# Adamtaranto/frisk

Hardware: NVIDIA B200
Metric: Gbp/s scaffold scored (k-mer count+window score) (higher is better)
Workload: dtype u4/u16/u64 counts + f64 scores

## Files before the change

### frisk_b200/csrc/frisk_tables.cu

```cuda
#include <cooperative_groups.h>
#include <cuda_runtime.h>
#include <math_constants.h>
#include <stdint.h>

#include <atomic>

#include "../../include/frisk_b200.h"
#include "frisk_internal.h"
#include "frisk_device.cuh"

namespace {

constexpr int kThreads = 1024;

__device__ __forceinline__ uint32_t revcomp_idx(uint32_t idx, int x) {
    uint32_t r = __brev(idx) >> (32 - 2 * x);
    r = ((r >> 1) & 0x55555555u) | ((r & 0x55555555u) << 1);
    return r ^ (0x55555555u & (pow4(x) - 1u));
}

__device__ __noinline__ void bg_wrapped(unsigned long long* __restrict__ fwd_k, uint32_t code, uint32_t old) {
    atomicAdd(&fwd_k[code], 65536ull);
    if (!(code & 1u))
        atomicAdd(&fwd_k[code | 1u], old == 0xffffffffu ? 65535ull : ~0ull);
}

__device__ __forceinline__ void bg_add(uint32_t* tab, unsigned long long* __restrict__ fwd_k, uint32_t code) {
    const uint32_t sh = (code & 1u) * 16u;
    const uint32_t old = atomicAdd(&tab[code >> 1], 1u << sh);
    if (((old >> sh) & 0xffffu) == 0xffffu) bg_wrapped(fwd_k, code, old);
}

__device__ __forceinline__ uint32_t bg_room(uint32_t old, uint32_t sh) { return ~(old | (0xffff0000u >> sh)); }

template <int K>
__global__ void __launch_bounds__(kThreads, 1)
bg_count_kernel(const uint32_t* __restrict__ codes, const uint32_t* __restrict__ inv, const uint32_t* __restrict__ low,
                uint64_t word_lo, uint64_t word_hi, int mask_host, unsigned long long* __restrict__ fwd,
                uint32_t* __restrict__ partial, const unsigned long long* __restrict__ d_range) {
    constexpr uint32_t NB = pow4(K);
    constexpr uint32_t NW = NB / 2u;
    extern __shared__ __align__(16) uint32_t tab[];
    if (d_range) { word_lo = d_range[0]; word_hi = d_range[1]; }
    const uint64_t n_words = word_hi - word_lo;
    const uint64_t per = (n_words + gridDim.x - 1) / gridDim.x;
    const uint64_t w0 = word_lo + per * blockIdx.x;
    uint64_t w1 = w0 + per;
    if (w1 > word_hi) w1 = word_hi;
    const bool use_low = mask_host && low != nullptr;
    unsigned long long* fwd_k = fwd + lvl_off(K);

    for (uint32_t b = threadIdx.x; b < NW; b += kThreads) tab[b] = 0;
    __syncthreads();
    for (uint64_t wd = w0 + threadIdx.x; wd < w1; wd += kThreads) {
        uint32_t m0 = __ldg(inv + wd), m1 = __ldg(inv + wd + 1);
        if (use_low) { m0 |= __ldg(low + wd); m1 |= __ldg(low + wd + 1); }
        const uint32_t c0 = __ldg(codes + 2 * wd), c1 = __ldg(codes + 2 * wd + 1), c2 = __ldg(codes + 2 * wd + 2);
        const bool all_valid = (m0 == 0u) && (K == 1 || (m1 >> ((33 - K) & 31)) == 0u);
        if (all_valid) {
            uint32_t olds[32], room = 0xffffffffu;
#pragma unroll
            for (int p = 0; p < 32; ++p) {
                const uint32_t code = (p < 16 ? __funnelshift_l(c1, c0, 2 * p) : __funnelshift_l(c2, c1, 2 * (p - 16)))
                                      >> (32 - 2 * K);
                const uint32_t sh = (code & 1u) * 16u;
                olds[p] = atomicAdd(&tab[code >> 1], 1u << sh);
                room = min(room, bg_room(olds[p], sh));
            }
            if (room == 0u) {
#pragma unroll 1
                for (int p = 0; p < 32; ++p) {
                    const uint32_t code = (p < 16 ? __funnelshift_l(c1, c0, 2 * p) : __funnelshift_l(c2, c1, 2 * (p - 16)))
                                          >> (32 - 2 * K);
                    uint32_t old = 0;
#pragma unroll
                    for (int q = 0; q < 32; ++q) if (q == p) old = olds[q];
                    if (bg_room(old, (code & 1u) * 16u) == 0u) bg_wrapped(fwd_k, code, old);
                }
            }
        } else {
#pragma unroll 4
            for (int p = 0; p < 32; ++p) {
                const uint32_t code = (p < 16 ? __funnelshift_l(c1, c0, 2 * p) : __funnelshift_l(c2, c1, 2 * (p - 16)))
                                      >> (32 - 2 * K);
                const int v = min(__clz(__funnelshift_l(m1, m0, p)), K);
                if (v == K) bg_add(tab, fwd_k, code);
                else if (v > 0) atomicAdd(&fwd[lvl_off(v) + (code >> (2 * (K - v)))], 1ull);
            }
        }
    }
    __syncthreads();
    if (partial) {
        uint32_t* dst = partial + (size_t)blockIdx.x * NW;
        if constexpr (NW >= 4u * kThreads) {
            for (uint32_t b = threadIdx.x * 4u; b < NW; b += kThreads * 4u)
                *reinterpret_cast<uint4*>(dst + b) = *reinterpret_cast<const uint4*>(tab + b);
        } else {
            for (uint32_t b = threadIdx.x; b < NW; b += kThreads) dst[b] = tab[b];
        }
    } else {
        for (uint32_t b = threadIdx.x; b < NW; b += kThreads) {
            const uint32_t c = tab[b];
            if (c & 0xffffu) atomicAdd(&fwd_k[2u * b], (unsigned long long)(c & 0xffffu));
            if (c >> 16) atomicAdd(&fwd_k[2u * b + 1u], (unsigned long long)(c >> 16));
        }
    }
}

template <int K>
__global__ void __launch_bounds__(256)
bg_reduce_kernel(const uint32_t* __restrict__ partial, int n_parts, unsigned long long* __restrict__ fwd) {
    constexpr uint32_t NW = pow4(K) / 2u;
    __shared__ unsigned long long acc[8][32][2];
    const uint32_t lane = threadIdx.x & 31u, warp = threadIdx.x >> 5;
    const uint32_t w = blockIdx.x * 32u + lane;
    unsigned long long lo = 0, hi = 0;
    if (w < NW) {
#pragma unroll 4
        for (int c = (int)warp; c < n_parts; c += 8) {
            const uint32_t v = partial[(size_t)c * NW + w];
            lo += v & 0xffffu;
            hi += v >> 16;
        }
    }
    acc[warp][lane][0] = lo; acc[warp][lane][1] = hi;
    __syncthreads();
    if (warp == 0 && w < NW) {
#pragma unroll
        for (int j = 1; j < 8; ++j) { lo += acc[j][lane][0]; hi += acc[j][lane][1]; }
        if (lo) fwd[lvl_off(K) + 2u * w] += lo;
        if (hi) fwd[lvl_off(K) + 2u * w + 1u] += hi;
    }
}

struct LocalFwd {
    const unsigned long long* p;
    const long long* space_dev = nullptr;
    __device__ __forceinline__ unsigned long long operator()(uint32_t i) const { return p[i]; }
    __device__ __forceinline__ void arrive_and_wait() const {}
    __device__ __forceinline__ long long space(long long by_value) const { return space_dev ? *space_dev : by_value; }
};
using frisk_internal::kMaxPeers;
struct PeerFwd {
    const unsigned long long* p[kMaxPeers];
    unsigned long long* flags[kMaxPeers];
    int n, rank;
    unsigned long long epoch;
    __device__ __forceinline__ long long space(long long by_value) const { return by_value; }
    __device__ __forceinline__ unsigned long long operator()(uint32_t i) const {
        unsigned long long v[kMaxPeers];
#pragma unroll
        for (int q = 0; q < kMaxPeers; ++q) v[q] = q < n ? __ldcv(p[q] + i) : 0ull;
        unsigned long long s = 0;
#pragma unroll
        for (int q = 0; q < kMaxPeers; ++q) s += v[q];
        return s;
    }
    __device__ __forceinline__ void arrive_and_wait() const {
        if (epoch == 0) return;
        if (blockIdx.x == 0 && (int)threadIdx.x < n) {
            __threadfence_system();
            asm volatile("st.release.sys.global.u64 [%0], %1;" ::"l"(flags[threadIdx.x] + rank), "l"(epoch) : "memory");
        }
        if (threadIdx.x == 0) {
            const long long t0 = clock64();
            for (int q = 0; q < n; ++q) {
                unsigned long long seen;
                do {
                    asm volatile("ld.acquire.sys.global.u64 %0, [%1];" : "=l"(seen) : "l"(flags[rank] + q) : "memory");
                    if (seen < epoch && clock64() - t0 > 20000000000ll) __trap();
                } while (seen < epoch);
            }
        }
        __syncthreads();
    }
};

template <int K, typename Fwd>
__device__ __forceinline__ void forward_totals_body(const Fwd& fwd, unsigned long long* __restrict__ tables,
                                                    unsigned long long* __restrict__ valid_kmax, uint32_t root,
                                                    unsigned long long (*lvl)[256], unsigned long long* red) {
    constexpr int R = K > 4 ? K - 4 : 0;
    const uint32_t t = threadIdx.x;
    uint32_t n = pow4(K - R);
    constexpr int LV = K - (R > 1 ? R : 1);
    unsigned long long own[LV > 0 ? LV : 1];
    unsigned long long v = 0;
    if (t < n) v = fwd(lvl_off(K) + root * n + t);
    {
        uint32_t m = n;
#pragma unroll
        for (int i = 0; i < LV; ++i) {
            m >>= 2;
            own[i] = (t < m) ? fwd(lvl_off(K - 1 - i) + root * m + t) : 0ull;
        }
    }
    if (t < n) {
        tables[lvl_off(K) + root * n + t] = v;
        lvl[0][t] = v;
    }
    unsigned long long local = v;
    for (int o = 16; o; o >>= 1) local += __shfl_xor_sync(kFull, local, o);
    if ((t & 31) == 0) red[t >> 5] = local;
    __syncthreads();
    if (t == 0 && valid_kmax) {
        unsigned long long sum = 0;
        for (int w = 0; w < 8; ++w) sum += red[w];
        if (sum) atomicAdd(valid_kmax, sum);
    }
    int cur = 0;
#pragma unroll
    for (int i = 0; i < LV; ++i) {
        const int x = K - 1 - i;
        n >>= 2;
        if (t < n) {
            const unsigned long long* ch = &lvl[cur][4 * t];
            const unsigned long long f = own[i] + ch[0] + ch[1] + ch[2] + ch[3];
            tables[lvl_off(x) + root * n + t] = f;
            lvl[cur ^ 1][t] = f;
        }
        cur ^= 1;
        __syncthreads();
    }
}

template <int K, typename Fwd>
__global__ void __launch_bounds__(256)
forward_totals_kernel(const Fwd fwd, unsigned long long* __restrict__ tables,
                      unsigned long long* __restrict__ valid_kmax) {
    __shared__ unsigned long long lvl[2][256];
    __shared__ unsigned long long red[8];
    fwd.arrive_and_wait();
    forward_totals_body<K, Fwd>(fwd, tables, valid_kmax, blockIdx.x, lvl, red);
}

template <int K, typename Fwd>
__device__ __forceinline__ void forward_low_body(const Fwd& fwd, unsigned long long* __restrict__ tables) {
    constexpr int R = K > 4 ? K - 4 : 0;
    const uint32_t t = threadIdx.x;
    unsigned long long own[R > 1 ? R - 1 : 1];
#pragma unroll
    for (int x = R - 1; x >= 1; --x) own[x - 1] = (t < pow4(x)) ? fwd(lvl_off(x) + t) : 0ull;
#pragma unroll
    for (int x = R - 1; x >= 1; --x) {
        if (t < pow4(x)) {
            const unsigned long long* ch = tables + lvl_off(x + 1) + 4 * t;
            tables[lvl_off(x) + t] = own[x - 1] + __ldcg(ch) + __ldcg(ch + 1) + __ldcg(ch + 2) + __ldcg(ch + 3);
        }
        __syncthreads();
    }
}

template <int K, typename Fwd>
__global__ void __launch_bounds__(64)
forward_low_kernel(const Fwd fwd, unsigned long long* __restrict__ tables) {
    forward_low_body<K, Fwd>(fwd, tables);
}

template <int K>
__device__ __forceinline__ void symmetrise_entry(unsigned long long* __restrict__ tables, uint32_t i) {
    int x = 1;
#pragma unroll
    for (int y = 2; y <= K; ++y) x += (i >= lvl_off(y));
    const uint32_t b = i - lvl_off(x);
    const uint32_t r = revcomp_idx(b, x);
    if (b < r) {
        const unsigned long long sum = __ldcg(tables + i) + __ldcg(tables + lvl_off(x) + r);
        tables[i] = sum;
        tables[lvl_off(x) + r] = sum;
    } else if (b == r) {
        tables[i] = 2ull * __ldcg(tables + i);
    }
}

template <int K>
__global__ void __launch_bounds__(256)
symmetrise_kernel(unsigned long long* __restrict__ tables) {
    const uint32_t i = blockIdx.x * 256 + threadIdx.x;
    if (i < lvl_off(K + 1)) symmetrise_entry<K>(tables, i);
}

template <int K>
__device__ __forceinline__ void genome_ivom_entry(const unsigned long long* __restrict__ tables, int kmin, long long space,
                                                  double2* __restrict__ ig, uint32_t kappa) {
    double num = 0.0;
    unsigned long long den = 0;
    bool bad = false;
#pragma unroll
    for (int x = 1; x <= K; ++x) {
        if (x < kmin) continue;
        const unsigned long long c = __ldcg(tables + lvl_off(x) + (kappa >> (2 * (K - x))));
        const long long d = (space - (long long)(x - 1)) * 2;
        if (d == 0) bad = true;
        const double q = (double)pow4(x) / (double)d;
        const double cd = (double)c;
        num = fma(q, cd * cd, num);
        den += c << (2 * x);
        if (x == kmin && c == 0) bad = true;
    }
    double v = bad ? CUDART_NAN : num / (double)den;
    ig[kappa] = make_double2(v, log2(v));
}

template <int K>
__global__ void genome_ivom_kernel(const unsigned long long* __restrict__ tables, int kmin, long long space,
                                   double2* __restrict__ ig) {
    const uint32_t kappa = blockIdx.x * blockDim.x + threadIdx.x;
    if (kappa < pow4(K)) genome_ivom_entry<K>(tables, kmin, space, ig, kappa);
}

template <int K, typename Fwd>
__global__ void __launch_bounds__(256)
finalize_ivom_kernel(const Fwd fwd, unsigned long long* __restrict__ tables, unsigned long long* __restrict__ valid_kmax,
                     int kmin, long long space, double2* __restrict__ ig) {
    namespace cg = cooperative_groups;
    cg::grid_group grid = cg::this_grid();
    constexpr int R = K > 4 ? K - 4 : 0;
    __shared__ unsigned long long lvl[2][256];
    __shared__ unsigned long long red[8];
    fwd.arrive_and_wait();
    for (uint32_t root = blockIdx.x; root < pow4(R); root += gridDim.x) {
        forward_totals_body<K, Fwd>(fwd, tables, valid_kmax, root, lvl, red);
        __syncthreads();
    }
    grid.sync();
    if (R > 1) {
        if (blockIdx.x == 0) forward_low_body<K, Fwd>(fwd, tables);
        grid.sync();
    }
    const uint32_t gtid = blockIdx.x * 256 + threadIdx.x, gstride = gridDim.x * 256;
    for (uint32_t i = gtid; i < lvl_off(K + 1); i += gstride) symmetrise_entry<K>(tables, i);
    grid.sync();
    const long long sp = fwd.space(space);
    for (uint32_t kappa = gtid; kappa < pow4(K); kappa += gstride) genome_ivom_entry<K>(tables, kmin, sp, ig, kappa);
}

using frisk_internal::check_k;
using frisk_internal::sm_count_cached;
#define CK(call) FRISK_CK(call)

template <int K>
int launch_background(const uint32_t* codes, const uint32_t* inv, const uint32_t* low, uint64_t w_lo, uint64_t w_hi,
                      int mask_host, uint64_t* fwd, cudaStream_t st, const unsigned long long* d_range = nullptr) {
    constexpr uint32_t NB = pow4(K);
    constexpr uint32_t NW = NB / 2u;
    const size_t smem = (size_t)NW * 4;
    CK(cudaFuncSetAttribute(bg_count_kernel<K>, cudaFuncAttributeMaxDynamicSharedMemorySize, (int)smem));
    const uint64_t n_words = w_hi - w_lo;
    int grid = sm_count_cached();
    if (grid <= 0) return FRISK_E_NO_DEVICE;
    const uint64_t want = (n_words + 2047) / 2048;
    if ((uint64_t)grid > want) grid = want ? (int)want : 1;
    uint32_t* partial = nullptr;
    if (NB >= 4096u && grid > 1) {
        int rc = frisk_internal::pool_ready();
        if (rc) return rc;
        CK(cudaMallocAsync((void**)&partial, (size_t)grid * NW * sizeof(uint32_t), st));
    }
    bg_count_kernel<K><<<grid, kThreads, smem, st>>>(codes, inv, low, w_lo, w_hi, mask_host,
                                                      reinterpret_cast<unsigned long long*>(fwd), partial, d_range);
    if (partial) {
        bg_reduce_kernel<K><<<(NW + 31) / 32, 256, 0, st>>>(partial, grid, reinterpret_cast<unsigned long long*>(fwd));
        CK(cudaFreeAsync(partial, st));
    }
    CK(cudaGetLastError());
    return FRISK_OK;
}

template <int K, typename Fwd>
int launch_finalize(const Fwd f, int symmetric, uint64_t* tables, uint64_t* valid, cudaStream_t st) {
    constexpr int R = K > 4 ? K - 4 : 0;
    auto t = reinterpret_cast<unsigned long long*>(tables);
    if (valid) CK(cudaMemsetAsync(valid, 0, sizeof(uint64_t), st));
    forward_totals_kernel<K, Fwd><<<pow4(R), 256, 0, st>>>(f, t, reinterpret_cast<unsigned long long*>(valid));
    if (R > 1) forward_low_kernel<K, Fwd><<<1, 64, 0, st>>>(f, t);
    if (symmetric) symmetrise_kernel<K><<<(lvl_off(K + 1) + 255) / 256, 256, 0, st>>>(t);
    CK(cudaGetLastError());
    return FRISK_OK;
}

template <int K, typename Fwd>
int launch_finalize_ivom(Fwd f, int kmin, int64_t space, uint64_t* tables, uint64_t* valid, double* ig, cudaStream_t st) {
    auto kern = finalize_ivom_kernel<K, Fwd>;
    static std::atomic<int> cached[64];
    int dev = 0;
    CK(cudaGetDevice(&dev));
    int per_sm = cached[dev & 63].load(std::memory_order_acquire);
    if (per_sm == 0) {
        CK(cudaOccupancyMaxActiveBlocksPerMultiprocessor(&per_sm, kern, 256, 0));
        if (per_sm > 0) cached[dev & 63].store(per_sm, std::memory_order_release);
    }
    const int sms = sm_count_cached();
    if (sms <= 0) return FRISK_E_NO_DEVICE;
    if (per_sm < 1) return FRISK_E_UNSUPPORTED;
    int grid = sms * (per_sm > 2 ? 2 : per_sm);
    if (valid) CK(cudaMemsetAsync(valid, 0, sizeof(uint64_t), st));
    unsigned long long* t = reinterpret_cast<unsigned long long*>(tables);
    unsigned long long* v = reinterpret_cast<unsigned long long*>(valid);
    long long sp = (long long)space;
    double2* g = reinterpret_cast<double2*>(ig);
    void* args[] = {(void*)&f, (void*)&t, (void*)&v, (void*)&kmin, (void*)&sp, (void*)&g};
    CK(cudaLaunchCooperativeKernel((const void*)kern, dim3((unsigned)grid), dim3(256), args, 0, st));
    return FRISK_OK;
}

template <int K>
int launch_genome_ivom(const uint64_t* tables, int kmin, int64_t space, double* ig, cudaStream_t st) {
    const uint32_t n = pow4(K);
    const int bs = 256;
    genome_ivom_kernel<K><<<(n + bs - 1) / bs, bs, 0, st>>>(reinterpret_cast<const unsigned long long*>(tables), kmin,
                                                           (long long)space, reinterpret_cast<double2*>(ig));
    CK(cudaGetLastError());
    return FRISK_OK;
}

int peer_fwd(const uint64_t* const* d_fwd_peers, uint64_t* const* d_flag_peers, int rank, int world, uint64_t epoch, PeerFwd* f) {
    if (world > kMaxPeers) return FRISK_E_UNSUPPORTED;
    f->n = world;
    f->rank = rank;
    f->epoch = d_flag_peers ? epoch : 0;
    for (int q = 0; q < kMaxPeers; ++q) { f->p[q] = nullptr; f->flags[q] = nullptr; }
    for (int q = 0; q < world; ++q) {
        if (!d_fwd_peers[q] || (d_flag_peers && !d_flag_peers[q])) return FRISK_E_INVALID;
        f->p[q] = reinterpret_cast<const unsigned long long*>(d_fwd_peers[q]);
        if (d_flag_peers) f->flags[q] = reinterpret_cast<unsigned long long*>(d_flag_peers[q]);
    }
    return FRISK_OK;
}

}

int frisk_internal::finalize_ivom(const uint64_t* d_fwd, const uint64_t* const* d_fwd_peers, uint64_t* const* d_flag_peers, int rank,
                                  int world, uint64_t epoch, int kmin, int kmax, int64_t space, const long long* space_dev,
                                  uint64_t* tables, uint64_t* valid, double* ig, cudaStream_t st) {
    int rc;
    if (kmax > FRISK_B200_FAST_K) {
        if (world > 0 || space_dev) return FRISK_E_UNSUPPORTED;
        if ((rc = frisk_internal::general_finalize(d_fwd, kmax, 1, tables, valid, st))) return rc;
        return frisk_internal::general_genome_ivom(tables, kmin, kmax, space, ig, st);
    }
    if (world == 0) {
        const LocalFwd f{reinterpret_cast<const unsigned long long*>(d_fwd), space_dev};
        DISPATCH_K(kmax, (launch_finalize_ivom<K, LocalFwd>(f, kmin, space, tables, valid, ig, st)));
    }
    if (space_dev) return FRISK_E_UNSUPPORTED;
    PeerFwd f;
    if ((rc = peer_fwd(d_fwd_peers, d_flag_peers, rank, world, epoch, &f))) return rc;
    DISPATCH_K(kmax, (launch_finalize_ivom<K, PeerFwd>(f, kmin, space, tables, valid, ig, st)));
}

extern "C" {

int frisk_b200_background(const uint32_t* d_codes, const uint32_t* d_inv, const uint32_t* d_low, uint64_t first_base,
                          uint64_t last_base, int kmax, int mask_host, uint64_t* d_fwd, void* stream) {
    if (!d_codes || !d_inv || !d_fwd || (first_base & 31) || (last_base & 31) || last_base < first_base)
        return FRISK_E_INVALID;
    int rc = check_k(1, kmax);
    if (rc) return rc;
    if (last_base == first_base) return FRISK_OK;
    cudaStream_t st = (cudaStream_t)stream;
    if (kmax > FRISK_B200_FAST_K)
        return frisk_internal::general_background(d_codes, d_inv, d_low, first_base >> 5, last_base >> 5, kmax, mask_host, d_fwd, st);
    DISPATCH_K(kmax, launch_background<K>(d_codes, d_inv, d_low, first_base >> 5, last_base >> 5, mask_host, d_fwd, st));
}

}

int frisk_internal::background_device_range(const uint32_t* codes, const uint32_t* inv, const uint32_t* low,
                                            const unsigned long long* d_word_range, uint64_t words_hint, int kmax, int mask_host,
                                            uint64_t* fwd, cudaStream_t st) {
    if (!codes || !inv || !fwd || !d_word_range) return FRISK_E_INVALID;
    int rc = check_k(1, kmax);
    if (rc) return rc;
    if (kmax > FRISK_B200_FAST_K) return FRISK_E_UNSUPPORTED;
    DISPATCH_K(kmax, launch_background<K>(codes, inv, low, 0, words_hint ? words_hint : 1, mask_host, fwd, st, d_word_range));
}

extern "C" {

int frisk_b200_finalize_tables(const uint64_t* d_fwd, int kmax, int symmetric, uint64_t* d_tables, uint64_t* d_valid_kmax,
                               void* stream) {
    if (!d_fwd || !d_tables) return FRISK_E_INVALID;
    int rc = check_k(1, kmax);
    if (rc) return rc;
    cudaStream_t st = (cudaStream_t)stream;
    if (kmax > FRISK_B200_FAST_K) return frisk_internal::general_finalize(d_fwd, kmax, symmetric, d_tables, d_valid_kmax, st);
    const LocalFwd f{reinterpret_cast<const unsigned long long*>(d_fwd)};
    DISPATCH_K(kmax, (launch_finalize<K, LocalFwd>(f, symmetric, d_tables, d_valid_kmax, st)));
}

int frisk_b200_finalize_tables_peers(const uint64_t* const* d_fwd_peers, uint64_t* const* d_flag_peers, int rank, int world,
                                     uint64_t epoch, int kmax, int symmetric, uint64_t* d_tables, uint64_t* d_valid_kmax,
                                     void* stream) {
    if (!d_fwd_peers || !d_tables || world < 1 || rank < 0 || rank >= world) return FRISK_E_INVALID;
    if (d_flag_peers && epoch == 0) return FRISK_E_INVALID;
    int rc = check_k(1, kmax);
    if (rc) return rc;
    if (kmax > FRISK_B200_FAST_K) return FRISK_E_UNSUPPORTED;
    PeerFwd f;
    if ((rc = peer_fwd(d_fwd_peers, d_flag_peers, rank, world, epoch, &f))) return rc;
    cudaStream_t st = (cudaStream_t)stream;
    DISPATCH_K(kmax, (launch_finalize<K, PeerFwd>(f, symmetric, d_tables, d_valid_kmax, st)));
}

int frisk_b200_finalize_ivom(const uint64_t* d_fwd, const uint64_t* const* d_fwd_peers, uint64_t* const* d_flag_peers, int rank,
                             int world, uint64_t epoch, int kmin, int kmax, int64_t genome_space, uint64_t* d_tables,
                             uint64_t* d_valid_kmax, double* d_ig, void* stream) {
    if (!d_tables || !d_ig || (world == 0 && !d_fwd) || (world > 0 && (!d_fwd_peers || rank < 0 || rank >= world)))
        return FRISK_E_INVALID;
    if (world > 0 && d_flag_peers && epoch == 0) return FRISK_E_INVALID;
    int rc = check_k(kmin, kmax);
    if (rc) return rc;
    return frisk_internal::finalize_ivom(d_fwd, d_fwd_peers, d_flag_peers, rank, world, epoch, kmin, kmax, genome_space, nullptr,
                                         d_tables, d_valid_kmax, d_ig, (cudaStream_t)stream);
}

int frisk_b200_genome_ivom(const uint64_t* d_tables, int kmin, int kmax, int64_t genome_space, double* d_ig, void* stream) {
    if (!d_tables || !d_ig) return FRISK_E_INVALID;
    int rc = check_k(kmin, kmax);
    if (rc) return rc;
    cudaStream_t st = (cudaStream_t)stream;
    if (kmax > FRISK_B200_FAST_K) return frisk_internal::general_genome_ivom(d_tables, kmin, kmax, genome_space, d_ig, st);
    DISPATCH_K(kmax, launch_genome_ivom<K>(d_tables, kmin, genome_space, d_ig, st));
}

}
```

### frisk_b200/engine.py

```python
from __future__ import annotations

import ctypes as C
import sys
from dataclasses import dataclass, field
from typing import List, Optional, Sequence, Tuple, Union

import numpy as np

from . import _lib

SeqLike = Union[np.ndarray, bytes, str]


def _torch_loaded() -> bool:
    return "torch" in sys.modules


class DevBuf:

    def __init__(self, nbytes: int):
        p = C.c_void_p()
        _lib.check(_lib.lib().frisk_b200_device_alloc(C.byref(p), int(nbytes)), "frisk_b200_device_alloc")
        self._p, self.nbytes = p, int(nbytes)

# ... 507 lines not shown
        _lib.check(_lib.lib().frisk_b200_score(_ptr(dg.codes), _ptr(dg.inv), _ptr(dg.low), _ptr(d_off), _ptr(d_len), n,
                                               wins.max_len, _ptr(d_ig), kmin, kmax, int(rip), _ptr(d_rows),
                                               _ptr(d_status), _ptr(d_dump), _stream_ptr(dev)), "frisk_b200_score")
    return d_rows, d_status, d_dump


_SLOT_CACHE = {}


def feature_slots(kmin: int, kmax: int) -> Tuple[np.ndarray, int]:
    key = (kmin, kmax)
    if key not in _SLOT_CACHE:
        slot = np.zeros(_lib.table_size(1, kmax), np.int32)
        n = C.c_uint64(0)
        _lib.check(_lib.lib().frisk_b200_feature_slots(kmin, kmax, _ptr(slot), C.byref(n)), "frisk_b200_feature_slots")
        _SLOT_CACHE[key] = (slot, int(n.value))
    return _SLOT_CACHE[key]


def region_features(dg: DeviceGenome, off: np.ndarray, length: np.ndarray, kmin: int = 1, kmax: int = 6) -> np.ndarray:
    import torch
    _lib.require_device()
    slot, nf = feature_slots(kmin, kmax)
    n = len(off)
    dev = dg.device
    d_out = torch.empty((n, nf), dtype=torch.float64, device=dev)
    if n:
        d_off = torch.from_numpy(np.ascontiguousarray(off, np.uint64).view(np.int64)).to(dev)
        d_len = torch.from_numpy(np.ascontiguousarray(length, np.uint32).view(np.int32)).to(dev)
        d_slot = torch.from_numpy(slot).to(dev)
        with torch.cuda.device(dev):
            _lib.check(_lib.lib().frisk_b200_region_features(_ptr(dg.codes), _ptr(dg.inv), _ptr(d_off), _ptr(d_len), n, kmin, kmax,
                                                             _ptr(d_slot), nf, _ptr(d_out), _stream_ptr(dev)),
                       "frisk_b200_region_features")
    return d_out.cpu().numpy()


@dataclass
class HotPathResult:
    kmin: int
    kmax: int
    tables: np.ndarray
    meta: Tuple[int, int, int]
    names: List[str]
    coords: np.ndarray
    rows: np.ndarray
    status: np.ndarray
    n_candidates: int = 0
    win_index: np.ndarray = field(default_factory=lambda: np.zeros(0, np.int64))
    row_scaf: np.ndarray = field(default_factory=lambda: np.zeros(0, np.int64))
    win_tables: Optional[np.ndarray] = None
    collective: str = ""
    scaf_names: List[str] = field(default_factory=list)

    def tsv_body(self, with_rip: bool) -> bytes:
        n = len(self.rows)
        enc = [s.encode() for s in self.scaf_names]
        lens = np.array([len(b) for b in enc], dtype=np.uint32)
        offs = (np.cumsum(lens, dtype=np.uint64) - lens).astype(np.uint64)
        blob = np.frombuffer(b"".join(enc) or b"\0", dtype=np.uint8)
        row_name = np.ascontiguousarray(self.row_scaf, dtype=np.uint32)
        start = np.ascontiguousarray(self.coords[:, 0], dtype=np.int64)
        stop = np.ascontiguousarray(self.coords[:, 1], dtype=np.int64)
        rows = np.ascontiguousarray(self.rows, dtype=np.float64)
        nv = 5 if with_rip else 2
        cap = int(lens[row_name].sum()) + n * (44 + 26 * nv) + 16 if n else 16
        out = np.empty(cap, dtype=np.uint8)
        nb = C.c_uint64(0)
        _lib.check(_lib.lib().frisk_b200_format_rows(_ptr(blob), _ptr(offs), _ptr(lens), _ptr(row_name), _ptr(start), _ptr(stop),
                                                     _ptr(rows), n, nv, _ptr(out), cap, C.byref(nb), 0), "frisk_b200_format_rows")
        return out[:int(nb.value)].tobytes()

    def raise_reference_errors(self) -> None:
        bad = np.nonzero(self.status & (_lib.ROW_KLD_ZERODIV | _lib.ROW_GC_ZERODIV))[0]
        if bad.size:
            i = int(bad[0])
            raise ZeroDivisionError("window %s:%d-%d: float division by zero (reference F:437/F:136)"
                                    % (self.names[i], self.coords[i, 0], self.coords[i, 1]))
        bad = np.nonzero(self.status & _lib.ROW_LOG_DOMAIN)[0]
        if bad.size:
            raise ValueError("math domain error (reference F:470)")


def _slice_orders(tab: np.ndarray, kmin: int, kmax: int) -> np.ndarray:
    return tab[..., _lib.table_size(1, kmin - 1):_lib.table_size(1, kmax)] if kmin > 1 else tab[..., :_lib.table_size(1, kmax)]


def assemble(query: PackedGenome, host: PackedGenome, wins: WindowList, tables_1k: np.ndarray, valid_kmax: int,
             rows: np.ndarray, status: np.ndarray, kmin: int, kmax: int, dump: Optional[np.ndarray] = None,
             names: bool = True) -> HotPathResult:
    keep = (status & _lib.ROW_EXCLUDED) == 0
    n_all = len(status)
    if bool(keep.all()):
        idx = np.arange(n_all, dtype=np.int64)
        take = lambda a: np.array(a[:n_all], copy=True)
    else:
        idx = np.nonzero(keep)[0]
        take = lambda a: a[idx]
    want_names = bool(names)
    scaf = take(wins.scaf)
    names = [query.names[s] for s in scaf] if want_names else []
    if idx.size:
        coords = np.empty((idx.size, 2), np.int64)
        coords[:, 0] = take(wins.start)
        coords[:, 1] = take(wins.stop)
    else:
        coords = np.zeros((0, 2), np.int64)
    meta = (host.total_len, host.ex_max(kmax, valid_kmax), host.nn_total)
    wt = None
    if dump is not None:
        wt = _slice_orders(take(dump), kmin, kmax)
    return HotPathResult(kmin, kmax, _slice_orders(tables_1k, kmin, kmax).copy(), meta, names, coords,
                         take(rows), take(status).astype(np.uint32, copy=False), len(wins), idx, scaf.astype(np.int64), wt,
                         scaf_names=list(query.names) if want_names else query.names)


class Pipeline:

    def __init__(self, query: PackedGenome, host: Optional[PackedGenome] = None, kmin: int = 1, kmax: int = 8,
                 w: int = 5000, step: int = 2500, mask_host: bool = False, scaffolds_all: bool = False,
                 rip: bool = True, device="cuda:0", dump: bool = False, allreduce=None,
                 genome_space: Optional[int] = None, wins: Optional[WindowList] = None,
                 bg_range: Optional[Tuple[int, int]] = None, peers=None):
        import torch
        _lib.require_device()
        rc = 0 if 1 <= kmin <= kmax else _lib.E_INVALID
        if kmax > _lib.MAX_K:
            rc = _lib.E_UNSUPPORTED
        _lib.check(rc, "frisk_b200 Pipeline(kmin=%d, kmax=%d)" % (kmin, kmax))
        host = host if host is not None else query
        self.dq = query if isinstance(query, DeviceGenome) else DeviceGenome(query, device)
        self.dh = self.dq if host is query else (host if isinstance(host, DeviceGenome) else DeviceGenome(host, device))
        query, host = self.dq.host, self.dh.host
        self.query, self.host = query, host
        self.kmin, self.kmax, self.mask_host, self.rip = kmin, kmax, mask_host, rip
        self.allreduce = allreduce
        self.peers = peers if (peers is not None and peers.available) else None
        self.genome_space = self.host.genome_space if genome_space is None else int(genome_space)
        self.wins = wins if wins is not None else query.windows(w, step, scaffolds_all)
        self.bg_range = (0, host.padded_len - 32) if bg_range is None else (int(bg_range[0]), int(bg_range[1]))
        dev = self.dq.device
        self.device = dev
        n = len(self.wins)
        tsz = _lib.table_size(1, kmax)
        self.d_fwd = torch.zeros(tsz, dtype=torch.int64, device=dev)
        self.d_tables = torch.empty(tsz, dtype=torch.int64, device=dev)
        self.d_valid = torch.zeros(1, dtype=torch.int64, device=dev)
        self.d_ig = torch.empty(2 * 4 ** kmax, dtype=torch.float64, device=dev)
        self.d_rows = torch.empty((n, 5), dtype=torch.float64, device=dev)
        self.d_status = torch.empty(n, dtype=torch.int32, device=dev)
        self.d_dump = torch.empty((n, tsz), dtype=torch.int16, device=dev) if dump else None
        self.d_off = torch.from_numpy(self.wins.off.view(np.int64)).to(dev, non_blocking=True)
        self.d_len = torch.from_numpy(self.wins.length.view(np.int32)).to(dev, non_blocking=True)
        self.launches_per_step = 4

    def enqueue(self, marks=None) -> None:
        import torch
        L = _lib.lib()
        dev = self.device

        def mark():
            if marks is not None:
                ev = torch.cuda.Event(enable_timing=True)
                ev.record(torch.cuda.current_stream(dev))
                marks.append(ev)

        with torch.cuda.device(dev):
            st = _stream_ptr(dev)
            d_fwd = self.peers.local() if self.peers is not None else self.d_fwd
            mark()
            d_fwd.zero_()
            dh = self.dh
            _lib.check(L.frisk_b200_background(_ptr(dh.codes), _ptr(dh.inv), _ptr(dh.low), self.bg_range[0], self.bg_range[1],
                                               self.kmax, int(self.mask_host), _ptr(d_fwd), st), "frisk_b200_background")
            mark()
            space = self.genome_space
            if self.peers is not None:
                self.peers.finalize_ivom(self.kmin, self.kmax, int(space), self.d_tables, self.d_valid, self.d_ig, st)
            else:
                if self.allreduce is not None:
                    space = self.allreduce(self.d_fwd, space)
                _lib.check(L.frisk_b200_finalize_ivom(_ptr(self.d_fwd), None, None, 0, 0, 0, self.kmin, self.kmax, int(space),
                                                      _ptr(self.d_tables), _ptr(self.d_valid), _ptr(self.d_ig), st),
                           "frisk_b200_finalize_ivom")
            mark()
            n = len(self.wins)
            if n:
                dq = self.dq
                _lib.check(L.frisk_b200_score(_ptr(dq.codes), _ptr(dq.inv), _ptr(dq.low), _ptr(self.d_off), _ptr(self.d_len),
                                              n, self.wins.max_len, _ptr(self.d_ig), self.kmin, self.kmax, int(self.rip),
                                              _ptr(self.d_rows), _ptr(self.d_status), _ptr(self.d_dump), st),
                           "frisk_b200_score")
            mark()

    def step_from_host(self, out: "HostOutputs") -> "HostOutputs":
        import torch
        dev = self.device
        with torch.cuda.device(dev):
            for dg in ((self.dh,) if self.dh is self.dq else (self.dh, self.dq)):
                g = dg.host
                dg.codes.copy_(torch.from_numpy(g.codes.view(np.int32)), non_blocking=True)
                dg.inv.copy_(torch.from_numpy(g.inv.view(np.int32)), non_blocking=True)
                if dg.low is not None:
                    dg.low.copy_(torch.from_numpy(g.low.view(np.int32)), non_blocking=True)
            self.d_off.copy_(torch.from_numpy(self.wins.off.view(np.int64)), non_blocking=True)
            self.d_len.copy_(torch.from_numpy(self.wins.length.view(np.int32)), non_blocking=True)
            self.enqueue()
            n = len(self.wins)
            if n:
                torch.from_numpy(out.rows[:n]).copy_(self.d_rows, non_blocking=True)
                torch.from_numpy(out.status[:n].view(np.int32)).copy_(self.d_status, non_blocking=True)
            torch.from_numpy(out.tables.view(np.int64)).copy_(self.d_tables, non_blocking=True)
            torch.from_numpy(out.valid.view(np.int64)).copy_(self.d_valid, non_blocking=True)
            torch.cuda.current_stream(dev).synchronize()
        return out

    def result(self, names: bool = True) -> HotPathResult:
        import torch
        torch.cuda.synchronize(self.device)
        tables = self.d_tables.cpu().numpy().view(np.uint64)
        n = len(self.wins)
        if n >= (1 << 16):
            h_rows = _staging("rows", (n, 5), np.float64)
            h_stat = _staging("status", (n,), np.int32)
            torch.from_numpy(h_rows).copy_(self.d_rows, non_blocking=True)
            torch.from_numpy(h_stat).copy_(self.d_status, non_blocking=True)
            torch.cuda.synchronize(self.device)
            rows, status = h_rows, h_stat.view(np.uint32)
        else:
            rows = self.d_rows.cpu().numpy()
            status = self.d_status.cpu().numpy().view(np.uint32)
        dmp = self.d_dump.cpu().numpy().view(np.uint16) if self.d_dump is not None else None
        return assemble(self.query, self.host, self.wins, tables, int(self.d_valid.item()), rows, status,
                        self.kmin, self.kmax, dmp, names=names)


def run(query, host=None, kmin: int = 1, kmax: int = 8, w: int = 5000,
        step: int = 2500, mask_host: bool = False, scaffolds_all: bool = False, rip: bool = True,
        device="cuda:0", dump: bool = False, allreduce=None, genome_space: Optional[int] = None,
        wins: Optional[WindowList] = None) -> HotPathResult:
    pipe = Pipeline(query, host, kmin, kmax, w, step, mask_host, scaffolds_all, rip, device, dump, allreduce,
                    genome_space, wins)
    pipe.enqueue()
    return pipe.result()


def run_sweep(query, kmaxes: Sequence[int] = tuple(range(1, 9)), kmin: int = 1, w: int = 5000, step: int = 2500,
              mask_host: bool = False, scaffolds_all: bool = False, rip: bool = True, device="cuda:0", fused: bool = True):
    import torch
    _lib.require_device()
    if fused:
        sw = Sweep(query, kmaxes, kmin, w, step, mask_host, scaffolds_all, rip, device)
        if sw.fused:
            sw.enqueue()
            return sw.results()
        query = sw.dq
    dq = query if isinstance(query, DeviceGenome) else DeviceGenome(query, device)
    g = dq.host
    top = max(kmaxes)
    d_tables, _ = finalize(background(dq, top, mask_host), top)
    wins = g.windows(w, step, scaffolds_all)
    out = {}
    for k in sorted(set(int(x) for x in kmaxes)):
        if k < kmin:
            continue
        tsz = _lib.table_size(1, k)
        d_tab_k = d_tables[:tsz]
        d_ig = genome_ivom(d_tab_k, kmin, k, g.genome_space)
        d_rows, d_status, _ = score(dq, wins, d_ig, kmin, k, rip)
        torch.cuda.synchronize(dq.device)
        tables = d_tab_k.cpu().numpy().view(np.uint64)
        valid = int(tables[_lib.table_size(1, k - 1) if k > 1 else 0:].sum()) // 2
        out[k] = assemble(g, g, wins, tables, valid, d_rows.cpu().numpy(), d_status.cpu().numpy().view(np.uint32), kmin, k)
    return out


class Sweep:

    def __init__(self, query, kmaxes: Sequence[int] = tuple(range(1, 9)), kmin: int = 1, w: int = 5000, step: int = 2500,
                 mask_host: bool = False, scaffolds_all: bool = False, rip: bool = True, device="cuda:0", rank: int = 0,
                 world: int = 1, allreduce=None, fused: bool = True):
        import torch
        from . import dist as fdist
        _lib.require_device()
        self.dq = query if isinstance(query, DeviceGenome) else DeviceGenome(query, device)
        g = self.dq.host
        self.kmaxes = sorted(set(int(k) for k in kmaxes if int(k) >= kmin))
        self.kmin, self.mask_host, self.rip, self.top = kmin, mask_host, rip, max(self.kmaxes)
        self.allreduce = allreduce
        self.wins_all = g.windows(w, step, scaffolds_all)
        a, b = fdist.split_windows(self.wins_all.length, world)[rank]
        self.wins = self.wins_all.slice(a, b)
        self.bg_range = fdist.split_base_range(g.padded_len, world)[rank] if world > 1 else (0, g.padded_len - 32)
        dev = self.dq.device
        self.device = dev
        n = len(self.wins)
        tsz = _lib.table_size(1, self.top)
        self.d_fwd = torch.zeros(tsz, dtype=torch.int64, device=dev)
        self.d_tables = torch.empty(tsz, dtype=torch.int64, device=dev)
        self.d_valid = torch.zeros(1, dtype=torch.int64, device=dev)
        self.d_ig = {k: torch.empty(2 * 4 ** k, dtype=torch.float64, device=dev) for k in self.kmaxes}
        self.d_rows = {k: torch.empty((n, 5), dtype=torch.float64, device=dev) for k in self.kmaxes}
        self.d_status = {k: torch.empty(n, dtype=torch.int32, device=dev) for k in self.kmaxes}
        self.d_off = torch.from_numpy(self.wins.off.view(np.int64)).to(dev)
        self.d_len = torch.from_numpy(self.wins.length.view(np.int32)).to(dev)
        self.launches = 0
        self.fused = bool(fused) and self.kmaxes == list(range(1, 9)) and kmin == 1 and 0 < self.wins.max_len <= 8186
# ... 250 lines not shown
```

Baseline: 58.27.

## Fuse partial reduction into cooperative count kernel and drop extra launches

The background k-mer count kernel now launches cooperatively and, after writing per-block partial tables, does a grid sync and reduces the partials itself with vectorized uint4 loads, which replaces the separate bg_reduce kernel. The main loop software-prefetches the next word's masks and codes, and the overflow check uses a cheaper OR of the high bits. The forward-totals kernel writes per-root sums into scratch and reduces them after the grid sync, which removes the memset launch and the atomic on valid_kmax. Together these cut the launches per step from four to three. The cost is a grid-wide barrier inside the count kernel, plus reuse of the ig buffer as scratch.

Measured after the change: 58.68, median of 6. Within noise of the previous version (+0.7%).

```diff
diff --git a/frisk_b200/csrc/frisk_tables.cu b/frisk_b200/csrc/frisk_tables.cu
--- a/frisk_b200/csrc/frisk_tables.cu
+++ b/frisk_b200/csrc/frisk_tables.cu
@@ -32,6 +32,97 @@
 }
 
 __device__ __forceinline__ uint32_t bg_room(uint32_t old, uint32_t sh) { return ~(old | (0xffff0000u >> sh)); }
+
+struct BgWord { uint32_t m0, m1, c0, c1, c2; };
+
+__device__ __forceinline__ BgWord bg_load(const uint32_t* __restrict__ codes, const uint32_t* __restrict__ inv,
+                                          const uint32_t* __restrict__ low, bool use_low, uint64_t wd, uint64_t w1) {
+    BgWord w{0u, 0u, 0u, 0u, 0u};
+    if (wd < w1) {
+        w.m0 = __ldg(inv + wd); w.m1 = __ldg(inv + wd + 1);
+        if (use_low) { w.m0 |= __ldg(low + wd); w.m1 |= __ldg(low + wd + 1); }
+        w.c0 = __ldg(codes + 2 * wd); w.c1 = __ldg(codes + 2 * wd + 1); w.c2 = __ldg(codes + 2 * wd + 2);
+    }
+    return w;
+}
+
+template <int K>
+__device__ __forceinline__ void bg_count_word(const BgWord& w, uint32_t* tab, unsigned long long* __restrict__ fwd) {
+    const bool all_valid = (w.m0 == 0u) && (K == 1 || (w.m1 >> ((33 - K) & 31)) == 0u);
+    unsigned long long* fwd_k = fwd + lvl_off(K);
+    if (all_valid) {
+        uint32_t olds[32], seen = 0u;
+#pragma unroll
+        for (int p = 0; p < 32; ++p) {
+            const uint32_t code = (p < 16 ? __funnelshift_l(w.c1, w.c0, 2 * p) : __funnelshift_l(w.c2, w.c1, 2 * (p - 16)))
+                                  >> (32 - 2 * K);
+            olds[p] = atomicAdd(&tab[code >> 1], 1u << ((code & 1u) * 16u));
+            seen |= olds[p];
+        }
+        if (seen & 0x80008000u) {
+#pragma unroll 1
+            for (int p = 0; p < 32; ++p) {
+                const uint32_t code = (p < 16 ? __funnelshift_l(w.c1, w.c0, 2 * p) : __funnelshift_l(w.c2, w.c1, 2 * (p - 16)))
+                                      >> (32 - 2 * K);
+                uint32_t old = 0;
+#pragma unroll
+                for (int q = 0; q < 32; ++q) if (q == p) old = olds[q];
+                if (bg_room(old, (code & 1u) * 16u) == 0u) bg_wrapped(fwd_k, code, old);
+            }
+        }
+    } else {
+#pragma unroll 4
+        for (int p = 0; p < 32; ++p) {
+            const uint32_t code = (p < 16 ? __funnelshift_l(w.c1, w.c0, 2 * p) : __funnelshift_l(w.c2, w.c1, 2 * (p - 16)))
+                                  >> (32 - 2 * K);
+            const int v = min(__clz(__funnelshift_l(w.m1, w.m0, p)), K);
+            if (v == K) bg_add(tab, fwd_k, code);
+            else if (v > 0) atomicAdd(&fwd[lvl_off(v) + (code >> (2 * (K - v)))], 1ull);
+        }
+    }
+}
+
+constexpr int kRedGroups = kThreads / 64, kRedBatch = 5;
+template <int K>
+__device__ __forceinline__ void bg_reduce_partials(const uint32_t* __restrict__ partial, int n_parts,
+                                                   unsigned long long* __restrict__ fwd_k, uint32_t* acc) {
+    constexpr uint32_t NW = pow4(K) / 2u, NC = NW / 4u;
+    const uint32_t per = (NC + gridDim.x - 1) / gridDim.x;
+    const uint32_t c_lo = blockIdx.x * per, c_hi = min(c_lo + per, NC);
+    const uint32_t col = threadIdx.x & 63u, grp = threadIdx.x >> 6;
+    for (uint32_t c0 = c_lo; c0 < c_hi; c0 += 64u) {
+        const uint32_t c = c0 + col;
+        uint32_t s[8] = {0u, 0u, 0u, 0u, 0u, 0u, 0u, 0u};
+        if (c < c_hi) {
+            for (int p0 = (int)grp; p0 < n_parts; p0 += kRedGroups * kRedBatch) {
+                uint4 v[kRedBatch];
+#pragma unroll
+                for (int j = 0; j < kRedBatch; ++j) {
+                    const int p = min(p0 + j * kRedGroups, n_parts - 1);
+                    v[j] = __ldcg(reinterpret_cast<const uint4*>(partial + (size_t)p * NW) + c);
+                    if (p0 + j * kRedGroups >= n_parts) v[j] = make_uint4(0u, 0u, 0u, 0u);
+                }
+#pragma unroll
+                for (int j = 0; j < kRedBatch; ++j) {
+                    s[0] += v[j].x & 0xffffu; s[1] += v[j].x >> 16;
+                    s[2] += v[j].y & 0xffffu; s[3] += v[j].y >> 16;
+                    s[4] += v[j].z & 0xffffu; s[5] += v[j].z >> 16;
+                    s[6] += v[j].w & 0xffffu; s[7] += v[j].w >> 16;
+                }
+            }
+        }
+        __syncthreads();
+        *reinterpret_cast<uint4*>(&acc[grp * 512u + col * 8u]) = make_uint4(s[0], s[1], s[2], s[3]);
+        *reinterpret_cast<uint4*>(&acc[grp * 512u + col * 8u + 4u]) = make_uint4(s[4], s[5], s[6], s[7]);
+        __syncthreads();
+        if (threadIdx.x < 512u && c0 + (threadIdx.x >> 3) < c_hi) {
+            unsigned long long t = 0;
+#pragma unroll
+            for (int g = 0; g < kRedGroups; ++g) t += acc[g * 512u + threadIdx.x];
+            if (t) fwd_k[8u * c0 + threadIdx.x] += t;
+        }
+    }
+}
 
 template <int K>
 __global__ void __launch_bounds__(kThreads, 1)
@@ -52,42 +143,11 @@
 
     for (uint32_t b = threadIdx.x; b < NW; b += kThreads) tab[b] = 0;
     __syncthreads();
+    BgWord cur = bg_load(codes, inv, low, use_low, w0 + threadIdx.x, w1);
     for (uint64_t wd = w0 + threadIdx.x; wd < w1; wd += kThreads) {
-        uint32_t m0 = __ldg(inv + wd), m1 = __ldg(inv + wd + 1);
-        if (use_low) { m0 |= __ldg(low + wd); m1 |= __ldg(low + wd + 1); }
-        const uint32_t c0 = __ldg(codes + 2 * wd), c1 = __ldg(codes + 2 * wd + 1), c2 = __ldg(codes + 2 * wd + 2);
-        const bool all_valid = (m0 == 0u) && (K == 1 || (m1 >> ((33 - K) & 31)) == 0u);
-        if (all_valid) {
-            uint32_t olds[32], room = 0xffffffffu;
-#pragma unroll
-            for (int p = 0; p < 32; ++p) {
-                const uint32_t code = (p < 16 ? __funnelshift_l(c1, c0, 2 * p) : __funnelshift_l(c2, c1, 2 * (p - 16)))
-                                      >> (32 - 2 * K);
-                const uint32_t sh = (code & 1u) * 16u;
-                olds[p] = atomicAdd(&tab[code >> 1], 1u << sh);
-                room = min(room, bg_room(olds[p], sh));
-            }
-            if (room == 0u) {
-#pragma unroll 1
-                for (int p = 0; p < 32; ++p) {
-                    const uint32_t code = (p < 16 ? __funnelshift_l(c1, c0, 2 * p) : __funnelshift_l(c2, c1, 2 * (p - 16)))
-                                          >> (32 - 2 * K);
-                    uint32_t old = 0;
-#pragma unroll
-                    for (int q = 0; q < 32; ++q) if (q == p) old = olds[q];
-                    if (bg_room(old, (code & 1u) * 16u) == 0u) bg_wrapped(fwd_k, code, old);
-                }
-            }
-        } else {
-#pragma unroll 4
-            for (int p = 0; p < 32; ++p) {
-                const uint32_t code = (p < 16 ? __funnelshift_l(c1, c0, 2 * p) : __funnelshift_l(c2, c1, 2 * (p - 16)))
-                                      >> (32 - 2 * K);
-                const int v = min(__clz(__funnelshift_l(m1, m0, p)), K);
-                if (v == K) bg_add(tab, fwd_k, code);
-                else if (v > 0) atomicAdd(&fwd[lvl_off(v) + (code >> (2 * (K - v)))], 1ull);
-            }
-        }
+        const BgWord nxt = bg_load(codes, inv, low, use_low, wd + kThreads, w1);
+        bg_count_word<K>(cur, tab, fwd);
+        cur = nxt;
     }
     __syncthreads();
     if (partial) {
@@ -98,38 +158,16 @@
         } else {
             for (uint32_t b = threadIdx.x; b < NW; b += kThreads) dst[b] = tab[b];
         }
+        if constexpr (NB >= 4096u) {
+            cooperative_groups::this_grid().sync();
+            bg_reduce_partials<K>(partial, (int)gridDim.x, fwd_k, tab);
+        }
     } else {
         for (uint32_t b = threadIdx.x; b < NW; b += kThreads) {
             const uint32_t c = tab[b];
             if (c & 0xffffu) atomicAdd(&fwd_k[2u * b], (unsigned long long)(c & 0xffffu));
             if (c >> 16) atomicAdd(&fwd_k[2u * b + 1u], (unsigned long long)(c >> 16));
         }
-    }
-}
-
-template <int K>
-__global__ void __launch_bounds__(256)
-bg_reduce_kernel(const uint32_t* __restrict__ partial, int n_parts, unsigned long long* __restrict__ fwd) {
-    constexpr uint32_t NW = pow4(K) / 2u;
-    __shared__ unsigned long long acc[8][32][2];
-    const uint32_t lane = threadIdx.x & 31u, warp = threadIdx.x >> 5;
-    const uint32_t w = blockIdx.x * 32u + lane;
-    unsigned long long lo = 0, hi = 0;
-    if (w < NW) {
-#pragma unroll 4
-        for (int c = (int)warp; c < n_parts; c += 8) {
-            const uint32_t v = partial[(size_t)c * NW + w];
-            lo += v & 0xffffu;
-            hi += v >> 16;
-        }
-    }
-    acc[warp][lane][0] = lo; acc[warp][lane][1] = hi;
-    __syncthreads();
-    if (warp == 0 && w < NW) {
-#pragma unroll
-        for (int j = 1; j < 8; ++j) { lo += acc[j][lane][0]; hi += acc[j][lane][1]; }
-        if (lo) fwd[lvl_off(K) + 2u * w] += lo;
-        if (hi) fwd[lvl_off(K) + 2u * w + 1u] += hi;
     }
 }
 
@@ -179,7 +217,8 @@
 template <int K, typename Fwd>
 __device__ __forceinline__ void forward_totals_body(const Fwd& fwd, unsigned long long* __restrict__ tables,
                                                     unsigned long long* __restrict__ valid_kmax, uint32_t root,
-                                                    unsigned long long (*lvl)[256], unsigned long long* red) {
+                                                    unsigned long long (*lvl)[256], unsigned long long* red,
+                                                    unsigned long long* __restrict__ root_sums = nullptr) {
     constexpr int R = K > 4 ? K - 4 : 0;
     const uint32_t t = threadIdx.x;
     uint32_t n = pow4(K - R);
@@ -206,7 +245,8 @@
     if (t == 0 && valid_kmax) {
         unsigned long long sum = 0;
         for (int w = 0; w < 8; ++w) sum += red[w];
-        if (sum) atomicAdd(valid_kmax, sum);
+        if (root_sums) root_sums[root] = sum;
+        else if (sum) atomicAdd(valid_kmax, sum);
     }
     int cur = 0;
 #pragma unroll
@@ -318,12 +358,24 @@
     constexpr int R = K > 4 ? K - 4 : 0;
     __shared__ unsigned long long lvl[2][256];
     __shared__ unsigned long long red[8];
+    unsigned long long* root_sums = reinterpret_cast<unsigned long long*>(ig);
     fwd.arrive_and_wait();
     for (uint32_t root = blockIdx.x; root < pow4(R); root += gridDim.x) {
-        forward_totals_body<K, Fwd>(fwd, tables, valid_kmax, root, lvl, red);
+        forward_totals_body<K, Fwd>(fwd, tables, valid_kmax, root, lvl, red, valid_kmax ? root_sums : nullptr);
         __syncthreads();
     }
     grid.sync();
+    if (blockIdx.x == 0 && valid_kmax) {
+        unsigned long long v = 0;
+        for (uint32_t r = threadIdx.x; r < pow4(R); r += 256) v += __ldcg(root_sums + r);
+        for (int o = 16; o; o >>= 1) v += __shfl_xor_sync(kFull, v, o);
+        if ((threadIdx.x & 31) == 0) red[threadIdx.x >> 5] = v;
+        __syncthreads();
+        if (threadIdx.x == 0) {
+            for (int w = 1; w < 8; ++w) v += red[w];
+            *valid_kmax = v;
+        }
+    }
     if (R > 1) {
         if (blockIdx.x == 0) forward_low_body<K, Fwd>(fwd, tables);
         grid.sync();
@@ -344,7 +396,8 @@
                       int mask_host, uint64_t* fwd, cudaStream_t st, const unsigned long long* d_range = nullptr) {
     constexpr uint32_t NB = pow4(K);
     constexpr uint32_t NW = NB / 2u;
-    const size_t smem = (size_t)NW * 4;
+    constexpr size_t kRedBytes = (size_t)kRedGroups * 512u * 4u;
+    const size_t smem = (NB >= 4096u && (size_t)NW * 4 < kRedBytes) ? kRedBytes : (size_t)NW * 4;
     CK(cudaFuncSetAttribute(bg_count_kernel<K>, cudaFuncAttributeMaxDynamicSharedMemorySize, (int)smem));
     const uint64_t n_words = w_hi - w_lo;
     int grid = sm_count_cached();
@@ -357,13 +410,12 @@
         if (rc) return rc;
         CK(cudaMallocAsync((void**)&partial, (size_t)grid * NW * sizeof(uint32_t), st));
     }
-    bg_count_kernel<K><<<grid, kThreads, smem, st>>>(codes, inv, low, w_lo, w_hi, mask_host,
-                                                      reinterpret_cast<unsigned long long*>(fwd), partial, d_range);
-    if (partial) {
-        bg_reduce_kernel<K><<<(NW + 31) / 32, 256, 0, st>>>(partial, grid, reinterpret_cast<unsigned long long*>(fwd));
-        CK(cudaFreeAsync(partial, st));
-    }
-    CK(cudaGetLastError());
+    unsigned long long* f = reinterpret_cast<unsigned long long*>(fwd);
+    int mh = mask_host;
+    void* args[] = {(void*)&codes, (void*)&inv, (void*)&low, (void*)&w_lo, (void*)&w_hi, (void*)&mh, (void*)&f, (void*)&partial,
+                    (void*)&d_range};
+    CK(cudaLaunchCooperativeKernel((const void*)bg_count_kernel<K>, dim3((unsigned)grid), dim3(kThreads), args, smem, st));
+    if (partial) CK(cudaFreeAsync(partial, st));
     return FRISK_OK;
 }
 
@@ -394,7 +446,6 @@
     if (sms <= 0) return FRISK_E_NO_DEVICE;
     if (per_sm < 1) return FRISK_E_UNSUPPORTED;
     int grid = sms * (per_sm > 2 ? 2 : per_sm);
-    if (valid) CK(cudaMemsetAsync(valid, 0, sizeof(uint64_t), st));
     unsigned long long* t = reinterpret_cast<unsigned long long*>(tables);
     unsigned long long* v = reinterpret_cast<unsigned long long*>(valid);
     long long sp = (long long)space;
diff --git a/frisk_b200/engine.py b/frisk_b200/engine.py
--- a/frisk_b200/engine.py
+++ b/frisk_b200/engine.py
@@ -683,7 +683,7 @@
         self.d_dump = torch.empty((n, tsz), dtype=torch.int16, device=dev) if dump else None
         self.d_off = torch.from_numpy(self.wins.off.view(np.int64)).to(dev, non_blocking=True)
         self.d_len = torch.from_numpy(self.wins.length.view(np.int32)).to(dev, non_blocking=True)
-        self.launches_per_step = 4
+        self.launches_per_step = 3
 
     def enqueue(self, marks=None) -> None:
         import torch
```
